# MarcBerliner/PETLION.jl

Hardware: AMD Instinct MI355X
Metric: DFN full-discharge trajectories/sec (ensemble) (higher is better)
Workload: dtype f64

## Files before the change

### petlion.jl_amd/csrc/dfn_cell.h

```cpp
#pragma once
#include <hip/hip_runtime.h>
#include <type_traits>
#include "../../include/petlion_hip.h"

namespace pl {

#ifndef PL_DEV
#define PL_DEV __device__ inline
#endif

constexpr int WAVE = 64;
#ifndef PL_NP
#define PL_NP 10
#endif
#ifndef PL_NS
#define PL_NS 10
#endif
#ifndef PL_NN
#define PL_NN 10
#endif
#ifndef PL_NR
#define PL_NR 10
#endif
#ifndef PL_NRN
// ... 989 lines not shown
              S.sei.jsPS[ks] = -aAE; S.sei.jsPE[ks] = aAE;
              S.sei.jsJ[ks] = aAE * FAR * Rfilm; S.sei.jsJS[ks] = 1.0 + aAE * FAR * Rfilm;
              S.sei.jsF[ks] = aAE * FAR * jt * crkag;
              S.sei.jsI[ks] = cwexp * ci0F * pwCm1 * Ex;
            } else {
              S.sei.jsPS[ks] = 0.0; S.sei.jsPE[ks] = 0.0; S.sei.jsJ[ks] = 0.0; S.sei.jsJS[ks] = 1.0; S.sei.jsF[ks] = 0.0; S.sei.jsI[ks] = 0.0;
            }
          }
        }
      }
    }
  }
}

template <class M>
PL_DEV void iso_cs_rows_rowb(CellLDS<M>& S, const double* Y, const double* YP, double* Fo) {
  PL_MODEL(M);
  const int lane = lane_id();
  const CellConst& c = S.cc;
  const int q = lane >> 4, r = lane & 15, rc = r < NR ? r : NR - 1;
  double Mrow[NR];
  for (int k = 0; k < NR; k++) Mrow[k] = S.Mr[rc * NR + k];
  [[maybe_unused]] double MrowN[NR_EQ ? 1 : NR];
  if constexpr (!NR_EQ) for (int k = 0; k < NR; k++) MrowN[k] = S.Mr[S.mr_el(1) + rc * NR + k];
  int pp[CSD_PASS]; double acc[CSD_PASS], cv[CSD_PASS], jv[CSD_PASS], ypv[CSD_PASS];
#pragma unroll
  for (int pass = 0; pass < CSD_PASS; pass++) {
    const int p = pass * CSD_G + q; pp[pass] = p < NJ ? p : NJ - 1; acc[pass] = 0.0;
    const int rk = rc < nr_of(pp[pass]) ? rc : nr_of(pp[pass]) - 1;
    cv[pass] = Y[O_CS + cs_off(pp[pass]) + rk];
    jv[pass] = Y[O_J + pp[pass]];
    ypv[pass] = YP[O_CS + cs_off(pp[pass]) + rk];
  }
  csd_settle(cv);
  static_for<0, NR>([&](auto kc) {
    constexpr int k = decltype(kc)::value;
#pragma unroll
    for (int pass = 0; pass < CSD_PASS; pass++) {
      if constexpr (NR_EQ) rowb_fmac<k>(acc[pass], cv[pass], Mrow[k]);
      else rowb_fmac<k>(acc[pass], cv[pass], pp[pass] < NP ? Mrow[k] : MrowN[k]);
    }
  });
  const double kap_p = c.kap_p, kap_n = c.kap_n, bj_p = c.bj_p, bj_n = c.bj_n;
#pragma unroll
  for (int pass = 0; pass < CSD_PASS; pass++) {
    const int p = pass * CSD_G + q;
    double rhs = (p < NP ? kap_p : kap_n) * acc[pass];
    if (r == nr_of(pp[pass]) - 1) rhs += (p < NP ? bj_p : bj_n) * jv[pass];
    if (p < NJ && r < nr_of(pp[pass])) Fo[O_CS + cs_off(p) + r] = rhs - ypv[pass];
  }
}

template <class M>
PL_DEV void iso_cs_rows(CellLDS<M>& S, const LaneRegs& R, const double* Y, const double* YP, double* Fo) {
  PL_MODEL(M);
  if constexpr (PL_CSDPP<M>) { iso_cs_rows_rowb(S, Y, YP, Fo); return; }
  if constexpr (M::W2) { if (wave_id() != 1) return; }
  const int lane = lane_id();
  const CellConst& c = S.cc;
  const int r = lane % NR, g = lane < CS_LANES ? lane / NR : CS_G - 1;
  double Mrow[NR];
  for (int k = 0; k < NR; k++) Mrow[k] = S.Mr[r * NR + k];
  [[maybe_unused]] double MrowN[NR_EQ ? 1 : NR];
  if constexpr (!NR_EQ) for (int k = 0; k < NR; k++) MrowN[k] = S.Mr[S.mr_el(1) + r * NR + k];
  int pp[CS_PASS]; double acc[CS_PASS];
#pragma unroll
  for (int pass = 0; pass < CS_PASS; pass++) { const int p = pass * CS_G + g; pp[pass] = p < NJ ? p : NJ - 1; acc[pass] = 0.0; }
  double v[CS_PASS][NR], jv[CS_PASS], ypv[CS_PASS];
#pragma unroll
  for (int pass = 0; pass < CS_PASS; pass++) {
#pragma unroll
    for (int k = 0; k < NR; k++) v[pass][k] = Y[O_CS + cs_off(pp[pass]) + k];
    jv[pass] = Y[O_J + pp[pass]];
    ypv[pass] = YP[O_CS + cs_off(pp[pass]) + r];
  }
  const double kap_p = c.kap_p, kap_n = c.kap_n, bj_p = c.bj_p, bj_n = c.bj_n;
#pragma unroll
  for (int k = 0; k < NR; k++) {
#pragma unroll
    for (int pass = 0; pass < CS_PASS; pass++) {
      if constexpr (NR_EQ) acc[pass] += Mrow[k] * v[pass][k];
      else acc[pass] += (pp[pass] < NP ? Mrow[k] : MrowN[k]) * v[pass][k];
    }
  }
#pragma unroll
  for (int pass = 0; pass < CS_PASS; pass++) {
    const int p = pass * CS_G + g;
    double rhs = (p < NP ? kap_p : kap_n) * acc[pass];
    if (r == nr_of(p) - 1) rhs += (p < NP ? bj_p : bj_n) * jv[pass];
    if (lane < CS_LANES && p < NJ && r < nr_of(p)) Fo[O_CS + cs_off(p) + r] = rhs - ypv[pass];
  }
}

template <bool WANT_RES, bool WANT_JAC, class M>
PL_DEV void cell_node_pass(CellLDS<M>& S, const double* Y, const double* YP, double* Fo, int mode, double value) {
  if constexpr (M::THERMAL) thermal_node_pass<WANT_RES, WANT_JAC>(S, Y, YP, Fo, mode, value);
  else iso_node_pass<WANT_RES, WANT_JAC>(S, Y, YP, Fo, mode, value);
}
template <bool WANT_JAC = false, class M>
PL_DEV void cell_cs_rows(CellLDS<M>& S, const LaneRegs& R, const double* Y, const double* YP, double* Fo) {
  if constexpr (M::THERMAL) thermal_cs_rows<WANT_JAC>(S, S.tb, Y, YP, Fo);
  else if constexpr (M::SD == 0) iso_cs_rows(S, R, Y, YP, Fo);
}
template <class M>
PL_DEV void cell_residual(CellLDS<M>& S, const LaneRegs& R, const double* Y, const double* YP, double* Fo, int mode, double value) {
  PL_TICE(2);
  cell_node_pass<true, false>(S, Y, YP, Fo, mode, value);
  if constexpr (M::THERMAL) PL_SYNC();
  PL_TOCE(S, 2, 5);
  cell_cs_rows<false>(S, R, Y, YP, Fo);
  PL_SYNC();
  PL_TOCE(S, 2, 6);
}
template <class M>
PL_DEV void cell_res_jac(CellLDS<M>& S, const LaneRegs& R, const double* Y, const double* YP, double* Fo, int mode, double value) {
  { PL_TICD(); cell_node_pass<true, true>(S, Y, YP, Fo, mode, value); PL_TOCD(S, 0); }
  if constexpr (M::THERMAL) PL_SYNC();
  { PL_TICD(); cell_cs_rows<true>(S, R, Y, YP, Fo); PL_TOCD(S, 1); }
  PL_SYNC();
}

__device__ __forceinline__ void inv3(const double* A, double* B) {
  const double c00 = A[4] * A[8] - A[5] * A[7], c01 = A[5] * A[6] - A[3] * A[8], c02 = A[3] * A[7] - A[4] * A[6];
  const double det = A[0] * c00 + A[1] * c01 + A[2] * c02;
  const double id = pl_rcp(det);
  B[0] = c00 * id; B[1] = (A[2] * A[7] - A[1] * A[8]) * id; B[2] = (A[1] * A[5] - A[2] * A[4]) * id;
  B[3] = c01 * id; B[4] = (A[0] * A[8] - A[2] * A[6]) * id; B[5] = (A[2] * A[3] - A[0] * A[5]) * id;
  B[6] = c02 * id; B[7] = (A[1] * A[6] - A[0] * A[7]) * id; B[8] = (A[0] * A[4] - A[1] * A[3]) * id;
}

template <class M>
__device__ __forceinline__ void node_block(const CellLDS<M>& S, int i, double cj, bool alg_only, double* D) {
  PL_MODEL(M);
  const int sc = sec_of(i);
  const bool elec = sc != 1;
  const int jx = sc == 0 ? i : i - NS;
  if (alg_only) { D[0] = 1.0; D[1] = 0.0; D[2] = 0.0; D[3] = 0.0; }
  else { D[0] = S.ceD[i] - cj; D[1] = 0.0; D[2] = 0.0; D[3] = S.pcD[i]; }
  D[4] = S.peD[i]; D[5] = 0.0; D[6] = 0.0; D[7] = 0.0; D[8] = 1.0;
  if (elec) {
    const bool first = (i == 0) || (i == NP + NS), last = (i == NP - 1) || (i == NE - 1);
    D[8] = (first || last) ? -1.0 : -2.0;
    const double gc = S.nphi[0][i], ge = S.nphi[1][i], gs = S.nphi[2][i];
    const double fs = alg_only ? 0.0 : S.ceJ[i], fp = S.peJ[i], fq = S.psJ[jx];
    D[0] -= fs * gc; D[1] -= fs * ge; D[2] -= fs * gs;
    D[3] -= fp * gc; D[4] -= fp * ge; D[5] -= fp * gs;
    D[6] -= fq * gc; D[7] -= fq * ge; D[8] -= fq * gs;
  }
}

#define PL_NMS3(r, a0, b0, a1, b1, a2, b2) ((((r) - (a0) * (b0)) - (a1) * (b1)) - (a2) * (b2))
#define PL_PMS3(r, a0, b0, a1, b1, a2, b2) ((((r) + (a0) * (b0)) + (a1) * (b1)) + (a2) * (b2))
#define PL_NMS4(r, a0, b0, a1, b1, a2, b2, a3, b3) (((((r) - (a0) * (b0)) - (a1) * (b1)) - (a2) * (b2)) - (a3) * (b3))

constexpr int TW_MID = NE / 2, TW_BASE = 32;
constexpr int TW_FWD = NE - TW_MID;
__device__ __forceinline__ int tw_node(int lane) { return lane < TW_MID ? lane : ((lane >= TW_BASE && lane < TW_BASE + (NE - TW_MID)) ? NE - 1 - (lane - TW_BASE) : -1); }
__host__ __device__ constexpr int tw_lane(int node) { return node < TW_MID ? node : TW_BASE + (NE - 1 - node); }
__device__ __forceinline__ double l22_of(int n) { return (n > 0 && sec_of(n) != 1 && sec_of(n - 1) == sec_of(n)) ? 1.0 : 0.0; }
__device__ __forceinline__ double u22_of(int n) { return (n < NE - 1 && sec_of(n) != 1 && sec_of(n + 1) == sec_of(n)) ? 1.0 : 0.0; }

template <class M>
__device__ __forceinline__ void thomas_sweeps(const CellLDS<M>& S, bool alg_only, double& r0, double& r1, double& r2) {
// ... 178 lines not shown
    const double a11 = head ? 0.0 : (top ? peLi : peUi), a22 = head ? 0.0 : (top ? l22_of(i) : u22_of(i));
    const double b00 = (alg_only || head) ? 0.0 : (top ? ceUn : ceLn), b10 = (alg_only || head) ? 0.0 : (top ? pcUn : pcLn);
    const double b11 = head ? 0.0 : (top ? peUn : peLn), b22 = a22;
    for (int k = 0; k < 9; k++) { LDm[k] = 0.0; Dn[k] = D[k]; }
    inv3(D, Dinv);
#pragma unroll 1
    for (int it = 1; it < TW_FWD; it++) {
      double P[9];
      for (int k = 0; k < 9; k++) P[k] = shift_up1(Dinv[k]);
      for (int k = 0; k < 3; k++) {
        LDm[k] = a00 * P[k];
        LDm[3 + k] = a10 * P[k] + a11 * P[3 + k];
        LDm[6 + k] = a22 * P[6 + k];
      }
      for (int rr = 0; rr < 3; rr++) {
        Dn[rr * 3 + 0] = (D[rr * 3 + 0] - LDm[rr * 3 + 0] * b00) - LDm[rr * 3 + 1] * b10;
        Dn[rr * 3 + 1] = D[rr * 3 + 1] - LDm[rr * 3 + 1] * b11;
        Dn[rr * 3 + 2] = D[rr * 3 + 2] - LDm[rr * 3 + 2] * b22;
      }
      inv3(Dn, Dinv);
    }
    {
      double P[9], L2[9], Dm[9], Dmi[9];
      for (int k = 0; k < 9; k++) P[k] = lane_bcast(Dinv[k], TW_MID - 1);
      const double c00 = alg_only ? 0.0 : S.ceL[TW_MID], c10 = alg_only ? 0.0 : S.pcL[TW_MID], c11 = S.peL[TW_MID], c22 = l22_of(TW_MID);
      const double e00 = alg_only ? 0.0 : S.ceU[TW_MID - 1], e10 = alg_only ? 0.0 : S.pcU[TW_MID - 1], e11 = S.peU[TW_MID - 1], e22 = c22;
      for (int k = 0; k < 3; k++) { L2[k] = c00 * P[k]; L2[3 + k] = c10 * P[k] + c11 * P[3 + k]; L2[6 + k] = c22 * P[6 + k]; }
      for (int rr = 0; rr < 3; rr++) {
        Dm[rr * 3 + 0] = (Dn[rr * 3 + 0] - L2[rr * 3 + 0] * e00) - L2[rr * 3 + 1] * e10;
        Dm[rr * 3 + 1] = Dn[rr * 3 + 1] - L2[rr * 3 + 1] * e11;
        Dm[rr * 3 + 2] = Dn[rr * 3 + 2] - L2[rr * 3 + 2] * e22;
      }
      inv3(Dm, Dmi);
      if (nd == TW_MID) for (int k = 0; k < 9; k++) { Dinv[k] = Dmi[k]; S.LDmid[k] = PL_F32(L2[k]); }
    }
    if (act) for (int k = 0; k < 9; k++) { S.Dinv[k][i] = PL_F32(Dinv[k]); S.LD[k][i] = PL_F32(LDm[k]); }
  }
  PL_SYNC();
  PL_TOCD(S, 4);
  if (mode != PLH_MODE_I) {
    const int nd = tw_node(lane);
    const int il = nd >= 0 ? nd : 0;
    double r0 = nd >= 0 ? S.colI[0][il] : 0.0, r1 = nd >= 0 ? S.colI[1][il] : 0.0, r2 = nd >= 0 ? S.colI[2][il] : 0.0;
    thomas_sweeps(S, alg_only, r0, r1, r2);
    if (nd >= 0) { S.x2[0][nd] = r0; S.x2[1][nd] = r1; S.x2[2][nd] = r2; }
    const double vx = (mode == PLH_MODE_ETA_P) ? lane_bcast(r2, tw_lane(NP + NS)) - lane_bcast(r1, tw_lane(NP + NS)) : lane_bcast(r2, tw_lane(0)) - lane_bcast(r2, tw_lane(NE - 1));
    if (lane == 0) S.bord = (mode == PLH_MODE_P) ? S.ctrlJ[1] - S.ctrlJ[0] * vx : -vx;
    PL_SYNC();
  }
  PL_TOCD(S, 5);
}

template <class M>
PL_DEV void iso_solve(CellLDS<M>& S, LaneRegs& R, double* b, int mode, bool alg_only) {
  PL_MODEL(M);
  const int lane = lane_id();
  const CellConst& c = S.cc;
  const int r = lane % NR, g = lane / NR;
  PL_TICE(2);
  if constexpr (PL_CSDPP<M>) {
    if (!alg_only) {
      const int q = lane >> 4, rr = lane & 15, rc = rr < NR ? rr : NR - 1;
      double AP[NR], AN[NR];
#pragma unroll
      for (int k = 0; k < NR; k++) { AP[k] = S.Ainv[0][rc * NR + k]; AN[k] = S.Ainv[1][rc * NR + k]; }
      int pp[CSD_PASS]; double w[CSD_PASS], bc[CSD_PASS];
#pragma unroll
      for (int pass = 0; pass < CSD_PASS; pass++) {
        const int p = pass * CSD_G + q; pp[pass] = p < NJ ? p : NJ - 1; w[pass] = 0.0;
        const int rk = rc < nr_of(pp[pass]) ? rc : nr_of(pp[pass]) - 1;
        bc[pass] = b[O_CS + cs_off(pp[pass]) + rk];
      }
      csd_settle(bc);
      static_for<0, NR>([&](auto kc) {
        constexpr int k = decltype(kc)::value;
#pragma unroll
        for (int pass = 0; pass < CSD_PASS; pass++)
          rowb_fmac<k>(w[pass], bc[pass], (pass + 1) * CSD_G <= NP ? AP[k] : (pass * CSD_G >= NP ? AN[k] : (pp[pass] < NP ? AP[k] : AN[k])));
      });
#pragma unroll
      for (int pass = 0; pass < CSD_PASS; pass++) {
        const int p = pass * CSD_G + q;
        if (p < NJ && rr == nr_of(pp[pass]) - 1) S.w9[p] = w[pass];
        R.wreg[pass] = w[pass];
      }
    }
  } else
  if constexpr (M::SD == 0)
  if (!alg_only && (!M::W2 || wave_id() == 1)) {
    const int gg = lane < CS_LANES ? g : CS_G - 1;
    int pp[CS_PASS]; double w[CS_PASS];
#pragma unroll
    for (int pass = 0; pass < CS_PASS; pass++) { const int p = pass * CS_G + gg; pp[pass] = p < NJ ? p : NJ - 1; w[pass] = 0.0; }
    double AP[NR], AN[NR], bv[CS_PASS][NR];
#pragma unroll
    for (int k = 0; k < NR; k++) { AP[k] = S.Ainv[0][r * NR + k]; AN[k] = S.Ainv[1][r * NR + k]; }
#pragma unroll
    for (int pass = 0; pass < CS_PASS; pass++) {
#pragma unroll
      for (int k = 0; k < NR; k++) bv[pass][k] = b[O_CS + cs_off(pp[pass]) + k];
    }
#pragma unroll
    for (int k = 0; k < NR; k++) {
      if constexpr (GRID_DEFAULT) {
        w[0] += AP[k] * bv[0][k];
        w[1] += (pp[1] < NP ? AP[k] : AN[k]) * bv[1][k];
        w[2] += AN[k] * bv[2][k];
        w[3] += AN[k] * bv[3][k];
      } else {
#pragma unroll
        for (int pass = 0; pass < CS_PASS; pass++)
          w[pass] += ((pass + 1) * CS_G <= NP ? AP[k] : (pass * CS_G >= NP ? AN[k] : (pp[pass] < NP ? AP[k] : AN[k]))) * bv[pass][k];
      }
    }
// ... 178 lines not shown
    case JT_J_Q: return S.gcs[a] * c.csq[a < NP ? 0 : 1];
    case JT_J_CE: return S.gce[a];
    case JT_J_CS: return S.gcs[a];
    case JT_J_J: if constexpr (M::SEI) { if (a >= NP) return S.sei.jjJ[a - NP]; }
                 if constexpr (M::SD != 0) return -1.0 + S.gcs[a] * c.csj[a < NP ? 0 : 1];
                 return -1.0;
    case JT_J_PE: return S.gpe[a];
    case JT_J_PS: return S.gps[a];
    case JT_PE_CL: return S.pcL[a];
    case JT_PE_CD: return S.pcD[a];
    case JT_PE_CU: return S.pcU[a];
    case JT_PE_L: return S.peL[a];
    case JT_PE_D: return S.peD[a];
    case JT_PE_U: return S.peU[a];
    case JT_PE_J: return S.peJ[a];
    case JT_PS_L: return 1.0;
    case JT_PS_D: return bb ? -1.0 : -2.0;
    case JT_PS_U: return 1.0;
    case JT_PS_J: return S.psJ[a];
    case JT_PS_I: return a == 0 ? c.JI0 : c.JI29;
    case JT_CTRL_P1: return 1.0;
    case JT_CTRL_M1: return -1.0;
    case JT_CTRL_PA: return S.ctrlJ[0];
    case JT_CTRL_PB: return -S.ctrlJ[0];
    case JT_CTRL_PI: return S.ctrlJ[1];
    case JT_CE_JS: return S.ceJ[a];
    case JT_PE_JS: return S.peJ[a];
    case JT_PS_JS: return S.psJ[a];
  }
  if constexpr (M::SEI) {
    switch (t) {
      case JT_J_F: return S.sei.jjF[a];
      case JT_F_JS: return -c.Mrho;
      case JT_F_F: return -cj;
      case JT_SOH_JS: return S.sei.sohw[a];
      case JT_SOH_SOH: return -cj;
      case JT_JS_PS: return S.sei.jsPS[a];
      case JT_JS_PE: return S.sei.jsPE[a];
      case JT_JS_J: return S.sei.jsJ[a];
      case JT_JS_JS: return S.sei.jsJS[a];
      case JT_JS_F: return S.sei.jsF[a];
      case JT_JS_I: return S.sei.jsI[a];
    }
  }
  return 0.0;
}

template <class M>
PL_DEV void cell_factor(CellLDS<M>& S, LaneRegs& R, const Tables* __restrict__ tb, double cj, int mode, bool alg_only) {
  if constexpr (M::THERMAL) thermal_factor(S, R, tb, cj, mode, alg_only);
  else iso_factor(S, R, tb, cj, mode, alg_only);
}
template <class M>
PL_DEV void cell_solve(CellLDS<M>& S, LaneRegs& R, double* b, int mode, bool alg_only) {
  if constexpr (M::THERMAL) thermal_solve(S, R, S.tb, b, mode, alg_only);
  else iso_solve(S, R, b, mode, alg_only);
}
template <bool FROZEN = false, class M>
PL_DEV double jac_entry(const CellLDS<M>& S, const Tables* __restrict__ tb, unsigned w, double cj) {
  if constexpr (M::THERMAL) return thermal_jac_entry<FROZEN>(S, tb, w, cj);
  else return iso_jac_entry(S, tb, w, cj);
}

struct GenRow {
  const plh_run* run = nullptr;
  double* W = nullptr;
  double gv = 0.0, bord = 1.0;
  int gcol = 0, ng = 0;
  __device__ __forceinline__ bool on() const { return run != nullptr; }
  __device__ __forceinline__ int col(int k) const { return lane_bcast_i(gcol, k); }
  __device__ __forceinline__ double dot(const double* b, int first_col) const {
    double s = 0.0;
    for (int k = 0; k < ng; k++) { const int c = col(k); const double v = lane_bcast(gv, k); if (c >= first_col) s += v * b[c]; }
    return s;
  }
};
template <class M>
PL_DEV void gen_solve(CellLDS<M>& S, LaneRegs& R, double* b, bool alg_only, const GenRow& g) {
  PL_MODEL(M);
  const int lane = lane_id(), wv = wave_id();
  PL_XSYNC();
  const double rho = b[O_I];
  PL_XSYNC();
  if (lane == 0 && wv == 0) b[O_I] = 0.0;
  PL_XSYNC();
  cell_solve(S, R, b, PLH_MODE_I, alg_only);
  PL_XSYNC();
  const double xI = (rho - g.dot(b, alg_only ? NDIFF : 0)) / g.bord;
  PL_XSYNC();
  _Pragma("unroll") for (int k__ = 0; k__ < NTRIP; k__++) if (const int n = vrow<M>(k__, lane, wv); vokg<M>(k__, lane, wv) && (!alg_only || n >= NDIFF)) b[n] += xI * g.W[n];
  PL_XSYNC();
}

template <class M>
PL_DEV void cell_solve_refined(CellLDS<M>& S, LaneRegs& R, const Tables* __restrict__ tb, double* b, double* bsave, double cjf, int mode, bool alg_only, int nref, const GenRow* g = nullptr) {
  PL_MODEL(M);
  const int lane = lane_id();
  const bool twin = mode == PL_MODE_DT_TWIN;
  const int jm = g ? PLH_MODE_I : (twin ? PLH_MODE_DT : mode);
  const int* __restrict__ ptr = tb->csr_ptr[jm]; const unsigned* __restrict__ code = tb->csr_code[jm]; const unsigned short* __restrict__ col = tb->csr_col[jm];
  const double cj = alg_only ? 0.0 : cjf;
  double xr[NTRIP];
  const int wv = wave_id();
  _Pragma("unroll") for (int k__ = 0; k__ < NTRIP; k__++) if (const int n = vrow<M>(k__, lane, wv); vokg<M>(k__, lane, wv)) bsave[n] = b[n];
  PL_XSYNC();
  for (int it = 0; it <= nref; it++) {
    if (it > 0) {
      double rr[NTRIP];
      PL_XSYNC();
// ... 28 lines not shown
```

### petlion.jl_amd/csrc/dfn_integrate.h

```cpp
#pragma once
#include "dfn_cell.h"

namespace pl {

constexpr int NTRIP_MAX = (2 * NE + NJ * NR + 2 * NJ + 1 + (NT > 2 * NN + 1 ? NT : 2 * NN + 1) + WAVE - 1) / WAVE;
struct IdaScalars {
  double tn, hh, hused, cj, cjlast, cjold, cjratio, ss, rr, h0_forced, rtol, atol;
  double ew[NTRIP_MAX];
  double ph[4][NTRIP_MAX];
  double ee[NTRIP_MAX];
  double pa[NTRIP_MAX], pb[NTRIP_MAX];
  int kk, kused, knew, phase, ns, maxord;
  int nst;
};

enum GenFlag { GF_STOPS = 1, GF_FUNC = 2, GF_EXPR = 4, GF_REFINE = 8, GF_GENROW = 16, GF_SENS = 32 };

enum Cnt { C_STEPS, C_RES, C_JAC, C_FACT, C_SOLVE, C_NEWTON, C_ERRFAIL, C_CONVFAIL, C_SUMKP2, C_INIT };
struct Counters { int v[10]; };
__device__ __forceinline__ void cnt_add(Counters& c, int k, int v = 1) { c.v[k] += v; }

#define PHI_RD(j, n) ((M::PHI_LDS > MAXORD || (j) < M::PHI_LDS) ? S.phi[(M::PHI_LDS > MAXORD || (j) < M::PHI_LDS) ? (j) : 0][n] : ((j) == M::PHI_LDS ? I.ph[0][k__] : ((j) == M::PHI_LDS + 1 ? I.ph[1][k__] : ((j) == M::PHI_LDS + 2 ? I.ph[2][k__] : I.ph[3][k__]))))
#define PHI_WR(j, n, v) do { if (M::PHI_LDS > MAXORD || (j) < M::PHI_LDS) S.phi[(M::PHI_LDS > MAXORD || (j) < M::PHI_LDS) ? (j) : 0][n] = (v); \
                           else if ((j) == M::PHI_LDS) I.ph[0][k__] = (v); else if ((j) == M::PHI_LDS + 1) I.ph[1][k__] = (v); \
                           else if ((j) == M::PHI_LDS + 2) I.ph[2][k__] = (v); else I.ph[3][k__] = (v); } while (0)
#define EE(n) I.ee[k__]
template <class M> constexpr bool PHI_REGS = M::PHI_LDS <= MAXORD;
#ifdef PL_EXP_BRANCHY_PHI
constexpr bool PL_BRANCHY_PHI = true;
#else
constexpr bool PL_BRANCHY_PHI = false;
#endif
template <class M> constexpr bool PL_FLAT = M::PHI_LDS > MAXORD && !M::W2;
#if defined(PL_OLD_STEP_BOUNDARY) && !defined(PL_WAVE_EMU) && !defined(PL_PHASE_TIMERS)
#error "PL_OLD_STEP_BOUNDARY is for wave-emulator test builds and phase-timer profiling builds only"
#endif
constexpr size_t PL_TWO_CELLS_LDS_MAX = 26624;
#ifdef PL_OLD_STEP_BOUNDARY
template <int F, class M> constexpr bool PL_STEPB = false;
#else
template <int F, class M> constexpr bool PL_STEPB = F == 0 && PL_FLAT<M> && (sizeof(CellLDS<M>) > PL_TWO_CELLS_LDS_MAX);
#endif
struct StepPt { double I, dI, V, dV, ep, dep; };
template <class M>
__device__ __forceinline__ void step_pt_load(StepPt& pt, const double* Y, const double* YP) {
  PL_MODEL(M);
  pt.I = Y[O_I]; pt.dI = YP[O_I]; pt.V = Y[O_PS] - Y[O_PS + NJ - 1]; pt.dV = YP[O_PS] - YP[O_PS + NJ - 1];
  pt.ep = Y[O_PS + NP] - Y[O_PE + NP + NS]; pt.dep = YP[O_PS + NP] - YP[O_PE + NP + NS];
}
#define PL_TRIP_BCAST(v, n) lane_bcast((v)[(n) / WAVE], (n) % WAVE)
template <class M>
__device__ __forceinline__ void step_pt_regs(StepPt& pt, const double* y, const double* yp) {
  PL_MODEL(M);
  static_assert(!M::W2, "entry n lives in trip n / 64 of lane n % 64 only with one wave per cell");
  pt.I = PL_TRIP_BCAST(y, O_I); pt.dI = PL_TRIP_BCAST(yp, O_I);
  pt.V = PL_TRIP_BCAST(y, O_PS) - PL_TRIP_BCAST(y, O_PS + NJ - 1); pt.dV = PL_TRIP_BCAST(yp, O_PS) - PL_TRIP_BCAST(yp, O_PS + NJ - 1);
  pt.ep = PL_TRIP_BCAST(y, O_PS + NP) - PL_TRIP_BCAST(y, O_PE + NP + NS); pt.dep = PL_TRIP_BCAST(yp, O_PS + NP) - PL_TRIP_BCAST(yp, O_PE + NP + NS);
}
#define PL_VEC(n) _Pragma("unroll") for (int k__ = 0; k__ < NTRIP; k__++) if (const int n = vrow<M>(k__, lane, wave_id()); vok<M>(k__, lane, wave_id()))
#define PL_VECG(n) _Pragma("unroll") for (int k__ = 0; k__ < NTRIP; k__++) if (const int n = vrow<M>(k__, lane, wave_id()); vokg<M>(k__, lane, wave_id()))

template <class M>
__device__ __forceinline__ double wrms(const double* v, const double* w) {
  PL_MODEL(M);
  const int lane = lane_id();
  double s = 0.0;
  PL_VEC(n) { const double p = v[n] * w[n]; s += p * p; }
  return sqrt(wave_sum(s) * (1.0 / NST));
}

PL_DEV double tab_eval(const plh_run& r, double t) {
  const int n = r.n_tab; const double* tt = r.tab_t; const double* vv = r.tab_v;
  if (n <= 0) return 0.0;
  if (t < tt[0]) return vv[0];
  int lo = 0, hi = n;
  while (hi - lo > 1) { const int mid = (lo + hi) >> 1; if (tt[mid] <= t) lo = mid; else hi = mid; }
  const int k = lo;
  if (k == n - 1) return vv[n - 1];
  const double dt = tt[k + 1] - tt[k];
  return dt > 0.0 ? vv[k] + (vv[k + 1] - vv[k]) * ((t - tt[k]) / dt) : vv[k + 1];
}
#ifdef PL_CLOSURE_HEADER
#include PL_CLOSURE_HEADER
#endif
template <class M>
PL_DEV double prog_eval(CellLDS<M>& S, const double* __restrict__ ops, const double* __restrict__ args, int k0, int k1, double t, const double* Y, const double* YP) {
  double* st = S.xstk + PLH_EXPR_STACK * wave_id(); const double* th = S.theta_row; int sp = 0;
  for (int k = k0; k < k1; k++) {
    const int op = (int)ops[k]; const double a = args[k];
    if (op <= PLH_OP_THETA) {
      double v;
      switch (op) { case PLH_OP_CONST: v = a; break; case PLH_OP_T: v = t; break; case PLH_OP_Y: v = Y[(int)a]; break; case PLH_OP_YP: v = YP[(int)a]; break; default: v = th[(int)a]; }
      st[sp++] = v;
    } else if (op == PLH_OP_SELECT) { const double b = st[sp - 1], x = st[sp - 2], c = st[sp - 3]; sp -= 2; st[sp - 1] = c != 0.0 ? x : b; }
// ... 273 lines not shown
      PL_VEC(n) { const double q = p5[k__] * f5; p5[k__] = q; a[k__] += m5 * q; b[k__] += g5 * q; }
      if (r4) { PL_VEC(n) S.phi[4][n] = p4[k__]; }
      if (r5) { PL_VEC(n) S.phi[5][n] = p5[k__]; }
    }
    if (resc[1]) { PL_VEC(n) S.phi[1][n] = p[0][k__]; }
    if (resc[2]) { PL_VEC(n) S.phi[2][n] = p[1][k__]; }
    if (resc[3]) { PL_VEC(n) S.phi[3][n] = p[2][k__]; }
  } else {
  PL_VEC(n) { a[k__] = S.phi[0][n]; b[k__] = 0.0; }
  if constexpr (PHI_REGS<M> && !PL_BRANCHY_PHI) {
    _Pragma("unroll") for (int j = 1; j <= MAXORD; j++) {
      if (j < M::PHI_LDS) {
        const double g = S.ida_gamma[j];
        if (first && j >= I.ns) { const double bt = S.ida_beta[j]; PL_VEC(n) { const double p = S.phi[j][n] * bt; S.phi[j][n] = p; a[k__] += p; b[k__] += g * p; } }
        else PL_VEC(n) { const double p = S.phi[j][n]; a[k__] += p; b[k__] += g * p; }
      } else {
        const bool on = j <= I.kk;
        const double m = on ? 1.0 : 0.0, mg = on ? S.ida_gamma[j <= MAXORD ? j : 0] : 0.0, bt = (on && first && j >= I.ns) ? S.ida_beta[j] : 1.0;
        PL_VEC(n) { const double p = PHI_RD(j, n) * bt; PHI_WR(j, n, p); a[k__] += m * p; b[k__] += mg * p; }
      }
    }
  } else
  _Pragma("unroll") for (int j = 1; j <= MAXORD; j++) if (j <= I.kk) {
    const double g = S.ida_gamma[j];
    if (first && j >= I.ns) {
      const double bt = S.ida_beta[j];
      PL_VEC(n) { const double p = PHI_RD(j, n) * bt; PHI_WR(j, n, p); a[k__] += p; b[k__] += g * p; }
    } else PL_VEC(n) { const double p = PHI_RD(j, n); a[k__] += p; b[k__] += g * p; }
  }
  }
  PL_VEC(n) { const double e = EE(n); S.yy[n] = a[k__] + e; S.yp[n] = b[k__] + I.cj * e; if (M::PRED_REGS) { I.pa[k__] = a[k__]; I.pb[k__] = b[k__]; } }
  PL_XSYNC();
  PL_AMARK("form_iterate end");
}

template <int F, class M>
PL_DEV int ida_nls(CellLDS<M>& S, LaneRegs& R, const Tables* tb, IdaScalars& I, int mode, double value, int jac_every_step, Counters& cnt, int nref, const plh_run* xrun = nullptr,
                   double* xvalue = nullptr, GenRow* g = nullptr) {
  PL_MODEL(M);
  const int lane = lane_id();
  const double epsNewt = 0.33, toldel = 0.0001 * epsNewt;
  int callLSetup = 0;
  if (I.nst == 0) { I.cjold = I.cj; I.ss = 20.0; callLSetup = 1; }
  else {
    I.cjratio = pl_div(I.cj, I.cjold);
    const double temp1 = (1.0 - 0.25) / (1.0 + 0.25), temp2 = 1.0 / temp1;
    if (I.cjratio < temp1 || I.cjratio > temp2) callLSetup = 1;
    if (I.cj != I.cjlast) I.ss = 100.0;
    if (jac_every_step) callLSetup = 1;
  }
  PL_VEC(n) EE(n) = 0.0;
  PL_SYNC();
  int jcur = 0, ret = 0, m = 0; bool done = false; double oldnrm = 0.0;
  for (bool first = true;; first = false) {
    if constexpr (PL_STEPB<F, M>) { if (done) break; }
    { PL_TIC(); form_iterate(S, I, first); PL_TOC(S, PH_NEWTVEC); }
    if (done) break;
    if constexpr ((F & GF_EXPR) != 0) { if (xrun) { value = closure_input(S, *xrun, I.tn, S.yy, S.yp); *xvalue = value; } }
    if (callLSetup) {
      PL_TIC();
      cell_res_jac(S, R, S.yy, S.yp, S.delta, mode, value);
      bool genf = false;
      if constexpr ((F & GF_GENROW) != 0) { if (g && g->on()) { genf = true; gen_factor(S, R, tb, I.cj, mode, false, *g, I.tn, S.yy, S.yp, S.yp); } }
      if (!genf) cell_factor(S, R, tb, I.cj, mode, false);
      cnt_add(cnt, C_RES); cnt_add(cnt, C_JAC); cnt_add(cnt, C_FACT);
      I.cjold = I.cj; I.cjratio = 1.0; I.ss = 20.0; jcur = 1; callLSetup = 0;
      PL_TOC(S, PH_JACFACT);
    } else {
      PL_TIC();
      cell_residual(S, R, S.yy, S.yp, S.delta, mode, value);
      cnt_add(cnt, C_RES);
      PL_TOC(S, PH_RES);
    }
    cnt_add(cnt, C_NEWTON); cnt_add(cnt, C_SOLVE);
    { PL_TIC();
    bool gens = false;
    if constexpr ((F & GF_GENROW) != 0) gens = g && g->on();
    if ((F & GF_REFINE) && nref > 0) cell_solve_refined(S, R, tb, S.delta, S.yp, I.cjold, mode, false, nref, gens ? g : nullptr);
    else if (gens) gen_solve(S, R, S.delta, false, *g);
    else cell_solve(S, R, S.delta, mode, false);
    PL_TOC(S, PH_SOLVE); }
    PL_TIC();
    const double sc = (I.cjratio != 1.0) ? -2.0 * pl_rcp(1.0 + I.cjratio) : -1.0;
    double s = 0.0;
    PL_VEC(n) { const double d = S.delta[n] * sc; EE(n) += d; const double p = d * EWT(n); s += p * p; }
    const double delnrm = pl_sqrt(block_sum<M>(S, s) * (1.0 / NST));
    PL_SYNC();
    ret = 2;
    if (m == 0) { oldnrm = delnrm; if (delnrm <= toldel) ret = 0; }
    else { const double q = pl_div(delnrm, oldnrm); const double rate = (m == 1) ? q : pow(q, 1.0 / m); if (rate > 0.9) ret = 1; else I.ss = pl_div(rate, 1.0 - rate); }
    if (ret == 2 && I.ss * delnrm <= epsNewt) ret = 0;
    if (!(delnrm == delnrm)) ret = 1;
    PL_TOC(S, PH_NEWTVEC);
    if (ret == 2) { m++; if (m < 4) continue; ret = 1; }
    if (ret == 1 && !jcur) { callLSetup = 1; m = 0; PL_VEC(n) EE(n) = 0.0; PL_SYNC(); continue; }
    done = true;
  }
  return ret;
}

template <class M>
PL_DEV int ida_test_error(CellLDS<M>& S, IdaScalars& I, double ck, double& err_k, double& err_km1) {
  PL_MODEL(M);
  const int lane = lane_id();
  const int kk = I.kk;
  PL_AMARK("test_error");
  double s0 = 0, s1 = 0, s2 = 0;
#ifdef PL_WAVE_EMU
  if (getenv("PL_EMU_TRACE_EE") && blockIdx.x == 0 && I.nst < atoi(getenv("PL_EMU_TRACE_EE"))) { PL_VEC(n) fprintf(stderr, "dev ee %d %d %.6e %.6e\n", I.nst + 1, n, EE(n), EE(n) * EWT(n)); }
#endif
  if constexpr (PL_FLAT<M>) {
    const int j1 = kk, j2 = kk > 1 ? kk - 1 : 0;
    double pk[NTRIP], pkm1[NTRIP];
    PL_VEC(n) { pk[k__] = S.phi[j1][n]; pkm1[k__] = S.phi[j2][n]; }
    PL_VEC(n) {
      const double w = EWT(n), e = EE(n);
      double p = e * w; s0 += p * p;
      const double d1 = pk[k__] + e; p = d1 * w; s1 += p * p;
      const double d2 = d1 + pkm1[k__]; p = d2 * w; s2 += p * p;
    }
  } else if constexpr (PHI_REGS<M>) {
    double pk[NTRIP], pkm1[NTRIP];
    PL_VEC(n) { pk[k__] = 0.0; pkm1[k__] = 0.0; }
    _Pragma("unroll") for (int j = 1; j <= MAXORD; j++) {
      if (j == kk && kk > 1) { PL_VEC(n) pk[k__] = PHI_RD(j, n); }
      else if (j == kk - 1 && kk > 2) { PL_VEC(n) pkm1[k__] = PHI_RD(j, n); }
    }
    PL_VEC(n) {
      const double w = EWT(n), e = EE(n);
      double p = e * w; s0 += p * p;
      if (kk > 1) { const double d1 = pk[k__] + e; p = d1 * w; s1 += p * p;
        if (kk > 2) { const double d2 = d1 + pkm1[k__]; p = d2 * w; s2 += p * p; } }
// ... 440 lines not shown
    double t0;
    if (new_run) { t0 = 0.0; if (!(Yinit && from_states)) cell_initial_guess(S, S.yy, SOC0); SOC = SOC0; }
    else t0 = nextafter(t_global, 1e300);
    double value = run.value, Iguess;
    const bool is_tab = (F & GF_FUNC) && (run.value_kind == PLH_VAL_TABLE || run.value_kind == PLH_VAL_EXPR);
    const bool is_fun = is_tab && run.mode != PLH_MODE_RES;
    if (is_tab) {
      value = run_input<F>(S, run, 0.0, S.yy, S.yp);
      if (mode == PLH_MODE_I) Iguess = value;
      else if (mode == PLH_MODE_P) Iguess = value / (cellV<M>(S.yy) * S.cc.I1C);
      else if (mode == PLH_MODE_RES) Iguess = have_prev ? prev_I : 1.0;
      else if (have_prev) Iguess = prev_I;
      else { const double OCV = cellV<M>(S.yy); Iguess = value > OCV ? 1.0 : -1.0; }
    } else
    if (dstate) {
      if (run.value_kind == PLH_VAL_HOLD) { value = 0.0; if (lane == 0 && wave_id() == 0) S.runc.value = 0.0; }
      Iguess = have_prev ? prev_I : 1.0;
    } else
    if (mode == PLH_MODE_I) {
      if (run.value_kind == PLH_VAL_HOLD) value = have_prev ? prev_I : 0.0;
      else if (run.value_kind == PLH_VAL_REST) value = 0.0;
      Iguess = value;
    } else if (mode == PLH_MODE_V) {
      if (run.value_kind == PLH_VAL_HOLD) { value = prev_V; Iguess = prev_V; }
      else if (have_prev && prev_I != 0.0) Iguess = prev_I;
      else { const double OCV = cellV<M>(S.yy); Iguess = value > OCV ? 1.0 : -1.0; }
    } else if (mode == PLH_MODE_P) {
      if (run.value_kind == PLH_VAL_HOLD) { value = prev_I * S.cc.I1C * prev_V; Iguess = prev_I; }
      else if (run.value_kind == PLH_VAL_REST) { value = 0.0; Iguess = 0.0; }
      else Iguess = value / (cellV<M>(S.yy) * S.cc.I1C);
    } else if (mode == PLH_MODE_ETA_P) {
      if (run.value_kind == PLH_VAL_HOLD) { value = prev_etap; Iguess = prev_I; }
      else if (have_prev) Iguess = prev_I;
      else { const double OCV = cellV<M>(S.yy); Iguess = value > OCV ? 1.0 : -1.0; }
    } else {
      if (run.value_kind == PLH_VAL_HOLD) value = 0.0;
      Iguess = have_prev ? prev_I : 1.0;
    }
    PL_XSYNC();
    if (lane == 0 && wave_id() == 0) S.yy[O_I] = Iguess;
    PL_XSYNC();
    GenRow grow;
    if constexpr ((F & GF_GENROW) != 0) { if (((run.value_kind == PLH_VAL_EXPR && run.n_dcol > 0) || dstate) && genW) { grow.run = &run; grow.W = genW; } }
    int flag = PLH_FLAG_RUNNING;
    plh_run_info ri; ri.flag = PLH_FLAG_RUNNING; ri.iterations = 0; ri.t_end = t_global; ri.V = 0; ri.I = 0; ri.SOC = SOC; ri.T_avg = T0;
    const bool continuation = !new_run;
    PrevVals pv; pv.frac = 1.0; pv.V = -1; pv.SOC = -1; pv.I = -1; pv.c_s_n = -1; pv.c_e_min = -1; pv.eta_pl = -1; pv.dfilm = -1; pv.T = -1; pv.g = -1;
    double tprev = 0.0, t = 0.0, t_prev_saved = t0; int iter = 1; bool stalled_once = false;
    double I_prev_pt = 0.0, t_restart = 0.0;
    [[maybe_unused]] StepPt spt;
#if defined(PL_WAVE_EMU) && !defined(PL_OLD_STEP_BOUNDARY)
    static_assert(!(F == 0 && PL_FLAT<M> && M::NST >= 301) || PL_STEPB<F, M>, "emulator build: the plain kernel of a 301-state model must take the new step boundary");
#endif
    [[maybe_unused]] double soc_nm1_s = 0.0, dt_step_s = 0.0, soc_n_s = 0.0;
    bool first_init = true, again = false, init_failed = false;
    [[maybe_unused]] int steps_since_restart = 2;
    auto init_block = [&]() -> bool {
    again = false;
    int ierr; { PL_TIC(); ierr = cell_init_consistent<F>(S, R, tb, S.yy, S.yp, S.delta, S.phi[1], mode, value, o.reltol_init, cnt, S.phi[0], o.refine,
                                                                       ((F & GF_EXPR) && (run.value_kind == PLH_VAL_EXPR || dstate)) ? &run : nullptr, t_restart, &grow); PL_TOC(S, PH_INIT); }
    if (ierr != 0) { if (first_init) init_failed = true; else flag = ierr; ri.flag = ierr; return false; }
    if constexpr ((F & GF_STOPS) != 0) { if (o.yp_alg_zero) { PL_VEC(n) if (n >= NDIFF) S.yp[n] = 0.0; PL_XSYNC(); } }
    ida_reinit(S, I, S.yy, S.yp, first_init ? (o.max_order > 0 && o.max_order <= MAXORD ? o.max_order : MAXORD) : I.maxord, t_restart);
    if (first_init) {
      first_init = false;
      save_pt(nout, t0, S.yy, SOC); nout++;
      check_stop<F>(S, run, o, 0.0, run.tf, S.yy, S.yp, SOC, pv, flag);
      PL_VECG(n) { Yprev[n] = S.yy[n]; YPprev[n] = S.yp[n]; }
      PL_SYNC();
      I_prev_pt = S.yy[O_I];
      if constexpr ((F & GF_SENS) != 0) sens_init(S, SX, mode, value, new_run, SOC0, o.reltol, o.abstol, nout - 1, run.value_kind == PLH_VAL_HOLD && have_prev, prev_V, prev_I);
    }
    return true;
    };
    bool init_ok = true;
    [[maybe_unused]] bool need_init = true;
    if constexpr ((F & GF_FUNC) == 0) init_ok = init_block();
    PL_TICH(pl_tl__);
    while (init_ok && flag == PLH_FLAG_RUNNING) {
      if constexpr ((F & GF_FUNC) != 0) {
        if (need_init) { need_init = false; if (!init_block()) break; if (flag != PLH_FLAG_RUNNING) break; }
      }
      double tret = t; tprev = t;
      double tstop_now;
      if constexpr ((F & GF_STOPS) != 0) tstop_now = next_tstop(o, t, continuation, run.tf);
      else tstop_now = (continuation && run.tf > 1.0 && t < 1.0) ? 1.0 : run.tf;
      if constexpr (M::W2) __syncthreads();
      PL_TOCH(S, pl_tl__, 1);
      const int sf = ida_step<F>(S, R, tb, I, tstop_now, tret, mode, value, o, cnt, (is_tab || dstate) ? &run : nullptr, &grow, &spt);
      if (sf != 0) {
        if (I.nst == 0 && !stalled_once) {
          stalled_once = true;
          PL_VECG(n) { S.yy[n] = Yprev[n]; S.yp[n] = YPprev[n]; }
          PL_XSYNC();
          ida_reinit(S, I, S.yy, S.yp, I.maxord); I.h0_forced = o.reltol; iter++; t = tprev;
          save_pt(nout, t + t0, S.yy, SOC); nout++;
          if constexpr ((F & GF_SENS) != 0) sens_repeat_point(S, SX, nout - 1);
          check_stop<F>(S, run, o, t, run.tf, S.yy, S.yp, SOC, pv, flag);
          continue;
        }
        if constexpr (PL_STEPB<F, M>) { static_assert(!PL_STEPB<F, M> || M::PRED_REGS, "the predictor of the last attempt must still be in registers"); form_iterate(S, I, false); }
        flag = sf; break;
      }
      iter++; t = tret;
      if constexpr ((F & GF_FUNC) != 0) steps_since_restart++;
      PL_TIC(); PL_TICE(3);
// ... 68 lines not shown
```

Measured before the change: 966,400.

## Fuse particle residual rows with the particle inverse solve in Newton iterations

In Newton iterations without a Jacobian refresh, a new chained routine computes the solid-concentration residual rows and applies the per-particle inverse directly in registers. The intermediate residual no longer has to be written to the delta vector and read back in the solve. The solve is told the particle part is already done (have_w) and skips its own Ainv pass. This saves LDS traffic and a pass of loads, at the cost of more registers live at once, and it is limited to large row-layout non-SEI models on the plain kernel.

```diff
diff --git a/petlion.jl_amd/csrc/dfn_cell.h b/petlion.jl_amd/csrc/dfn_cell.h
--- a/petlion.jl_amd/csrc/dfn_cell.h
+++ b/petlion.jl_amd/csrc/dfn_cell.h
@@ -1065,6 +1065,61 @@
 }
 
 template <class M>
+PL_DEV void iso_cs_chain_rowb(CellLDS<M>& S, LaneRegs& R, const double* Y, const double* YP) {
+  PL_MODEL(M);
+  static_assert(PL_CSDPP<M>, "row layout only");
+  const int lane = lane_id();
+  const CellConst& c = S.cc;
+  const int q = lane >> 4, r = lane & 15, rc = r < NR ? r : NR - 1;
+  double Mrow[NR], AP[NR], AN[NR];
+#pragma unroll
+  for (int k = 0; k < NR; k++) { Mrow[k] = S.Mr[rc * NR + k]; AP[k] = S.Ainv[0][rc * NR + k]; AN[k] = S.Ainv[1][rc * NR + k]; }
+  [[maybe_unused]] double MrowN[NR_EQ ? 1 : NR];
+  if constexpr (!NR_EQ) for (int k = 0; k < NR; k++) MrowN[k] = S.Mr[S.mr_el(1) + rc * NR + k];
+  const double kap_p = c.kap_p, kap_n = c.kap_n, bj_p = c.bj_p, bj_n = c.bj_n;
+  int pp[CSD_PASS]; double acc[CSD_PASS], cv[CSD_PASS], jv[CSD_PASS], ypv[CSD_PASS];
+#pragma unroll
+  for (int pass = 0; pass < CSD_PASS; pass++) {
+    const int p = pass * CSD_G + q; pp[pass] = p < NJ ? p : NJ - 1; acc[pass] = 0.0;
+    const int rk = rc < nr_of(pp[pass]) ? rc : nr_of(pp[pass]) - 1;
+    cv[pass] = Y[O_CS + cs_off(pp[pass]) + rk];
+    jv[pass] = Y[O_J + pp[pass]];
+    ypv[pass] = YP[O_CS + cs_off(pp[pass]) + rk];
+  }
+  csd_settle(cv);
+  static_for<0, NR>([&](auto kc) {
+    constexpr int k = decltype(kc)::value;
+#pragma unroll
+    for (int pass = 0; pass < CSD_PASS; pass++) {
+      if constexpr (NR_EQ) rowb_fmac<k>(acc[pass], cv[pass], Mrow[k]);
+      else rowb_fmac<k>(acc[pass], cv[pass], pp[pass] < NP ? Mrow[k] : MrowN[k]);
+    }
+  });
+  double f[CSD_PASS], w[CSD_PASS];
+#pragma unroll
+  for (int pass = 0; pass < CSD_PASS; pass++) {
+    const int p = pass * CSD_G + q;
+    double rhs = (p < NP ? kap_p : kap_n) * acc[pass];
+    if (r == nr_of(pp[pass]) - 1) rhs += (p < NP ? bj_p : bj_n) * jv[pass];
+    f[pass] = rhs - ypv[pass];
+    w[pass] = 0.0;
+  }
+  csd_settle(f);
+  static_for<0, NR>([&](auto kc) {
+    constexpr int k = decltype(kc)::value;
+#pragma unroll
+    for (int pass = 0; pass < CSD_PASS; pass++)
+      rowb_fmac<k>(w[pass], f[pass], (pass + 1) * CSD_G <= NP ? AP[k] : (pass * CSD_G >= NP ? AN[k] : (pp[pass] < NP ? AP[k] : AN[k])));
+  });
+#pragma unroll
+  for (int pass = 0; pass < CSD_PASS; pass++) {
+    const int p = pass * CSD_G + q;
+    if (p < NJ && r == nr_of(pp[pass]) - 1) S.w9[p] = w[pass];
+    R.wreg[pass] = w[pass];
+  }
+}
+
+template <class M>
 PL_DEV void iso_cs_rows(CellLDS<M>& S, const LaneRegs& R, const double* Y, const double* YP, double* Fo) {
   PL_MODEL(M);
   if constexpr (PL_CSDPP<M>) { iso_cs_rows_rowb(S, Y, YP, Fo); return; }
@@ -1115,13 +1170,13 @@
   if constexpr (M::THERMAL) thermal_cs_rows<WANT_JAC>(S, S.tb, Y, YP, Fo);
   else if constexpr (M::SD == 0) iso_cs_rows(S, R, Y, YP, Fo);
 }
-template <class M>
+template <bool CS_ROWS = true, class M>
 PL_DEV void cell_residual(CellLDS<M>& S, const LaneRegs& R, const double* Y, const double* YP, double* Fo, int mode, double value) {
   PL_TICE(2);
   cell_node_pass<true, false>(S, Y, YP, Fo, mode, value);
   if constexpr (M::THERMAL) PL_SYNC();
   PL_TOCE(S, 2, 5);
-  cell_cs_rows<false>(S, R, Y, YP, Fo);
+  if constexpr (CS_ROWS) cell_cs_rows<false>(S, R, Y, YP, Fo);
   PL_SYNC();
   PL_TOCE(S, 2, 6);
 }
@@ -1406,14 +1461,14 @@
 }
 
 template <class M>
-PL_DEV void iso_solve(CellLDS<M>& S, LaneRegs& R, double* b, int mode, bool alg_only) {
+PL_DEV void iso_solve(CellLDS<M>& S, LaneRegs& R, double* b, int mode, bool alg_only, bool have_w = false) {
   PL_MODEL(M);
   const int lane = lane_id();
   const CellConst& c = S.cc;
   const int r = lane % NR, g = lane / NR;
   PL_TICE(2);
   if constexpr (PL_CSDPP<M>) {
-    if (!alg_only) {
+    if (!alg_only && !have_w) {
       const int q = lane >> 4, rr = lane & 15, rc = rr < NR ? rr : NR - 1;
       double AP[NR], AN[NR];
 #pragma unroll
@@ -1698,9 +1753,13 @@
   else iso_factor(S, R, tb, cj, mode, alg_only);
 }
 template <class M>
-PL_DEV void cell_solve(CellLDS<M>& S, LaneRegs& R, double* b, int mode, bool alg_only) {
+PL_DEV void cell_solve(CellLDS<M>& S, LaneRegs& R, double* b, int mode, bool alg_only, bool have_w = false) {
   if constexpr (M::THERMAL) thermal_solve(S, R, S.tb, b, mode, alg_only);
-  else iso_solve(S, R, b, mode, alg_only);
+  else iso_solve(S, R, b, mode, alg_only, have_w);
+}
+template <class M>
+PL_DEV void cell_cs_chain(CellLDS<M>& S, LaneRegs& R, const double* Y, const double* YP) {
+  iso_cs_chain_rowb(S, R, Y, YP);
 }
 template <bool FROZEN = false, class M>
 PL_DEV double jac_entry(const CellLDS<M>& S, const Tables* __restrict__ tb, unsigned w, double cj) {
diff --git a/petlion.jl_amd/csrc/dfn_integrate.h b/petlion.jl_amd/csrc/dfn_integrate.h
--- a/petlion.jl_amd/csrc/dfn_integrate.h
+++ b/petlion.jl_amd/csrc/dfn_integrate.h
@@ -40,6 +40,14 @@
 template <int F, class M> constexpr bool PL_STEPB = false;
 #else
 template <int F, class M> constexpr bool PL_STEPB = F == 0 && PL_FLAT<M> && (sizeof(CellLDS<M>) > PL_TWO_CELLS_LDS_MAX);
+#endif
+#if defined(PL_OLD_NEWTON_PARTICLES) && !defined(PL_WAVE_EMU) && !defined(PL_PHASE_TIMERS)
+#error "PL_OLD_NEWTON_PARTICLES is for wave-emulator test builds and phase-timer profiling builds only"
+#endif
+#ifdef PL_OLD_NEWTON_PARTICLES
+template <int F, class M> constexpr bool PL_NEWTP = false;
+#else
+template <int F, class M> constexpr bool PL_NEWTP = F == 0 && PL_CSDPP<M> && !M::SEI && (sizeof(CellLDS<M>) > PL_TWO_CELLS_LDS_MAX);
 #endif
 struct StepPt { double I, dI, V, dV, ep, dep; };
 template <class M>
@@ -419,6 +427,7 @@
   PL_VEC(n) EE(n) = 0.0;
   PL_SYNC();
   int jcur = 0, ret = 0, m = 0; bool done = false; double oldnrm = 0.0;
+  [[maybe_unused]] bool have_w = false;
   for (bool first = true;; first = false) {
     if constexpr (PL_STEPB<F, M>) { if (done) break; }
     { PL_TIC(); form_iterate(S, I, first); PL_TOC(S, PH_NEWTVEC); }
@@ -433,9 +442,14 @@
       cnt_add(cnt, C_RES); cnt_add(cnt, C_JAC); cnt_add(cnt, C_FACT);
       I.cjold = I.cj; I.cjratio = 1.0; I.ss = 20.0; jcur = 1; callLSetup = 0;
       PL_TOC(S, PH_JACFACT);
+      if constexpr (PL_NEWTP<F, M>) have_w = false;
     } else {
       PL_TIC();
-      cell_residual(S, R, S.yy, S.yp, S.delta, mode, value);
+      if constexpr (PL_NEWTP<F, M>) {
+        { PL_TICE(2); cell_cs_chain(S, R, S.yy, S.yp); PL_TOCE(S, 2, 6); }
+        cell_residual<false>(S, R, S.yy, S.yp, S.delta, mode, value);
+        have_w = true;
+      } else cell_residual(S, R, S.yy, S.yp, S.delta, mode, value);
       cnt_add(cnt, C_RES);
       PL_TOC(S, PH_RES);
     }
@@ -445,6 +459,7 @@
     if constexpr ((F & GF_GENROW) != 0) gens = g && g->on();
     if ((F & GF_REFINE) && nref > 0) cell_solve_refined(S, R, tb, S.delta, S.yp, I.cjold, mode, false, nref, gens ? g : nullptr);
     else if (gens) gen_solve(S, R, S.delta, false, *g);
+    else if constexpr (PL_NEWTP<F, M>) cell_solve(S, R, S.delta, mode, false, have_w);
     else cell_solve(S, R, S.delta, mode, false);
     PL_TOC(S, PH_SOLVE); }
     PL_TIC();
@@ -991,6 +1006,9 @@
 #if defined(PL_WAVE_EMU) && !defined(PL_OLD_STEP_BOUNDARY)
     static_assert(!(F == 0 && PL_FLAT<M> && M::NST >= 301) || PL_STEPB<F, M>, "emulator build: the plain kernel of a 301-state model must take the new step boundary");
 #endif
+#if defined(PL_WAVE_EMU) && !defined(PL_OLD_NEWTON_PARTICLES)
+    static_assert(!(F == 0 && PL_CSDPP<M> && !M::SEI && M::NST >= 301) || PL_NEWTP<F, M>, "emulator build: the plain kernel of a 301-state row-layout model must take the fused particle chain");
+#endif
     [[maybe_unused]] double soc_nm1_s = 0.0, dt_step_s = 0.0, soc_n_s = 0.0;
     bool first_init = true, again = false, init_failed = false;
     [[maybe_unused]] int steps_since_restart = 2;
```

Result: faster. 980,600, median of 6 (+1.5%).
